# google/guetzli

Measured on AMD Instinct MI355X. Metric: MPix/s encoded at --quality 95, higher is better.
Workload: dtype f32+f64 (butteraugli), int32/int16 (DCT/quantize/entropy coding); 1 GPU; single 3840x2160 sRGB image, --quality 95 (BASELINE configs[2]), whole guetzli::Process per step (host RGB in, JPEG bytes out), 1 image per GPU per step; 12 timed steps after 5 warm-up between barrier + synchronise, max over ranks; images_per_gpu=1, steps=12, warmup=5, output_bytes=2895866

## Files before the change

guetzli_amd/csrc/api/chain.h:

```cpp
#pragma once

namespace {
static bool packed_blur(const gz_ctx* c) {
  if (c->cfg.blur_packed >= 0) return c->cfg.blur_packed != 0;
  return (size_t)c->w * c->h >= 1500000;
}
constexpr int kTileRows = 32;
constexpr int kSmallTileRows = 16;
static bool small_tiles(const gz_ctx* c) {
  if (c->cfg.tile_rows == 16) return true;
  if (c->cfg.tile_rows == 32) return false;
  return (size_t)c->w * c->h < 7000000;
}

template <int R, class Src, int NC>
int blur_h(gz_ctx* c, const SrcPack<Src, NC>& src, const PlanePack<NC>& dst,
           const BlurCfg& cfg) {
  if (cfg.r != R) { c->err = "blur radius mismatch"; return GZ_E_STATE; }
  const Taps<R> tp = taps_of<R>(cfg);
  const BorderScale bs = cfg.bx;
  const int w = c->w, h = c->h, pitch = c->pitch;
  if (packed_blur(c)) {
    dim3 grid(gz_div_up(c->w, HW), gz_div_up(c->h, HP), NC);
    GZ_LAUNCH((k_blur_h_pk<R, Src, NC>), grid, dim3(256), c->stream, src, dst, w, h, pitch, tp, bs, tp, bs);
  } else {
    dim3 grid(gz_div_up(c->w, HW), gz_div_up(c->h, HH), NC);
    GZ_LAUNCH((k_blur_h<R, Src, NC>), grid, dim3(256), c->stream, src, dst, w, h, pitch, tp, bs, tp, bs);
  }
  KCHK(c);
  return GZ_OK;
}

template <int R, int NC, class Post>
int blur_v(gz_ctx* c, const CPlanePack<NC>& src, const Post& post, const BlurCfg& cfg) {
  if (cfg.r != R) { c->err = "blur radius mismatch"; return GZ_E_STATE; }
  const Taps<R> tp = taps_of<R>(cfg);
  const BorderScale bs = cfg.by;
  const int w = c->w, h = c->h, pitch = c->pitch;
  const bool small = small_tiles(c);
  dim3 grid(gz_div_up(c->w, VW), gz_div_up(c->h, small ? kSmallTileRows : kTileRows));
  if (packed_blur(c)) {
    if (small) GZ_LAUNCH((k_blur_v_pk<R, NC, Post, kSmallTileRows>), grid, dim3(256), c->stream, src, post, w, h, pitch, tp, bs, tp, bs);
    else GZ_LAUNCH((k_blur_v_pk<R, NC, Post, kTileRows>), grid, dim3(256), c->stream, src, post, w, h, pitch, tp, bs, tp, bs);
  } else {
    if (small) GZ_LAUNCH((k_blur_v_compact<R, NC, Post, kSmallTileRows>), grid, dim3(256), c->stream, src, post, w, h, pitch, tp, bs, tp, bs);
    else GZ_LAUNCH((k_blur_v_compact<R, NC, Post, kTileRows>), grid, dim3(256), c->stream, src, post, w, h, pitch, tp, bs, tp, bs);
  }
  KCHK(c);
  return GZ_OK;
}

template <int R, class Src>
int blur_h_pair(gz_ctx* c, const SrcPack<Src, 2>& src, const PlanePack<2>& dst, const BlurCfg& cfg0,
                const BlurCfg& cfg1) {
  if (cfg0.r != R || cfg1.r != R) { c->err = "blur radius mismatch"; return GZ_E_STATE; }
  const Taps<R> t0 = taps_of<R>(cfg0), t1 = taps_of<R>(cfg1);
  const BorderScale b0 = cfg0.bx, b1 = cfg1.bx;
  const int w = c->w, h = c->h, pitch = c->pitch;
  if (packed_blur(c)) {
    dim3 grid(gz_div_up(c->w, HW), gz_div_up(c->h, HP), 2);
    GZ_LAUNCH((k_blur_h_pk<R, Src, 2, true>), grid, dim3(256), c->stream, src, dst, w, h, pitch, t0, b0, t1, b1);
  } else {
    dim3 grid(gz_div_up(c->w, HW), gz_div_up(c->h, HH), 2);
    GZ_LAUNCH((k_blur_h<R, Src, 2, true>), grid, dim3(256), c->stream, src, dst, w, h, pitch, t0, b0, t1, b1);
  }
  KCHK(c);
  return GZ_OK;
}
template <int R>
int blur_v_pair(gz_ctx* c, const CPlanePack<2>& src, const PostStore<2>& post, const BlurCfg& cfg0,
                const BlurCfg& cfg1) {
  if (cfg0.r != R || cfg1.r != R) { c->err = "blur radius mismatch"; return GZ_E_STATE; }
  const Taps<R> t0 = taps_of<R>(cfg0), t1 = taps_of<R>(cfg1);
  const BorderScale b0 = cfg0.by, b1 = cfg1.by;
  const int w = c->w, h = c->h, pitch = c->pitch;
  const bool small = small_tiles(c);
  dim3 grid(gz_div_up(c->w, VW), gz_div_up(c->h, small ? kSmallTileRows : kTileRows), 2);
  if (packed_blur(c)) {
    if (small) GZ_LAUNCH((k_blur_v_pk<R, 2, PostStore<2>, kSmallTileRows, true>), grid, dim3(256), c->stream, src, post, w, h, pitch, t0, b0, t1, b1);
    else GZ_LAUNCH((k_blur_v_pk<R, 2, PostStore<2>, kTileRows, true>), grid, dim3(256), c->stream, src, post, w, h, pitch, t0, b0, t1, b1);
  } else {
    if (small) GZ_LAUNCH((k_blur_v_compact<R, 2, PostStore<2>, kSmallTileRows, true>), grid, dim3(256), c->stream, src, post, w, h, pitch, t0, b0, t1, b1);
    else GZ_LAUNCH((k_blur_v_compact<R, 2, PostStore<2>, kTileRows, true>), grid, dim3(256), c->stream, src, post, w, h, pitch, t0, b0, t1, b1);
  }
  KCHK(c);
  return GZ_OK;
}

template <int R, int NC, class Src, class Post, bool BM = false>
int blur2d(gz_ctx* c, const SrcPack<Src, NC>& src, const Post& post, const BlurCfg& cfg,
           BlockMaxOut bm = BlockMaxOut{nullptr, nullptr, 0, nullptr}, int n_tiles = 0) {
  if (cfg.r != R) { c->err = "blur radius mismatch"; return GZ_E_STATE; }
  const Taps<R> tp = taps_of<R>(cfg);
  const BorderScale bx = cfg.bx, by = cfg.by;
  const int w = c->w, h = c->h, pitch = c->pitch;
  if (bm.tiles || (BM ? small_tiles(c) && (size_t)c->w * c->h < 1500000 : small_tiles(c))) {
    dim3 grid(gz_div_up(c->w, T2), gz_div_up(c->h, kSmallTileRows));
    if (bm.tiles) grid = dim3(n_tiles);
    GZ_LAUNCH((k_blur2d<R, NC, Src, Post, BM, kSmallTileRows>), grid, dim3(256), c->stream, src, post, w,
              h, pitch, tp, bx, by, bm);
  } else {
    dim3 grid(gz_div_up(c->w, T2), gz_div_up(c->h, kTileRows));
    if (bm.tiles) grid = dim3(n_tiles);
    GZ_LAUNCH((k_blur2d<R, NC, Src, Post, BM, kTileRows>), grid, dim3(256), c->stream, src, post, w,
              h, pitch, tp, bx, by, bm);
  }
  KCHK(c);
  return GZ_OK;
}

#define TRY(x) do { int rc_ = (x); if (rc_ != GZ_OK) return rc_; } while (0)

static int stage_reserve(gz_ctx* c, HostStage* st, size_t bytes, void** out) {
  if (!st->ev) HIPCHK(c, pool_event_create(&st->ev));
  if (st->busy) {
    HIPCHK(c, hipEventSynchronize(st->ev));
    st->busy = false;
  }
  if (bytes > st->cap) {
    if (st->h) (void)pool_host_free(st->h);
    st->h = nullptr;
    st->cap = 0;
    const size_t cap = bytes + bytes / 2 + 4096;
    HIPCHK(c, pool_host_malloc(&st->h, cap));
    st->cap = cap;
  }
  *out = st->h;
  return GZ_OK;
}
static int stage_sent(gz_ctx* c, HostStage* st, hipStream_t stream) {
  HIPCHK(c, hipEventRecord(st->ev, stream));
  st->busy = true;
  return GZ_OK;
}
static int result_buffer(gz_ctx* c, size_t bytes, void** out) {
  if (bytes > c->h_res_cap) {
    if (c->h_res) (void)pool_host_free(c->h_res);
    c->h_res = nullptr;
    c->h_res_cap = 0;
    const size_t cap = std::max<size_t>(bytes + bytes / 2, 1 << 16);
    HIPCHK(c, pool_host_malloc(&c->h_res, cap));
    c->h_res_cap = cap;
  }
  *out = c->h_res;
  return GZ_OK;
}
static void stage_free(HostStage* st) {
  if (st->ev) { (void)hipEventSynchronize(st->ev); pool_event_destroy(st->ev); }
  if (st->h) (void)pool_host_free(st->h);
  st->h = nullptr; st->ev = nullptr; st->cap = 0; st->busy = false;
}

int setup_blur_cfg(gz_ctx* c, BlurCfg* cfg, float sigma, float border_ratio) {
  make_taps_host(sigma, cfg);
  cfg->border_ratio = border_ratio;
  std::vector<float> xl, xh, yl, yh;
  border_scales_host(*cfg, c->w, &xl, &xh);
  border_scales_host(*cfg, c->h, &yl, &yh);
  const int r = cfg->r;
  if (cfg->d_scale == nullptr) HIPCHK(c, pool_malloc((void**)&cfg->d_scale, sizeof(float) * 4 * r));
  std::vector<float> all;
  all.insert(all.end(), xl.begin(), xl.end());
  all.insert(all.end(), xh.begin(), xh.end());
  all.insert(all.end(), yl.begin(), yl.end());
  all.insert(all.end(), yh.begin(), yh.end());
  HIPCHK(c, hipMemcpy(cfg->d_scale, all.data(), sizeof(float) * 4 * r, hipMemcpyHostToDevice));
  cfg->bx.lo = cfg->d_scale;
  cfg->bx.hi = cfg->d_scale + r;
  cfg->by.lo = cfg->d_scale + 2 * r;
  cfg->by.hi = cfg->d_scale + 3 * r;
  return GZ_OK;
}

int stage_opsin(gz_ctx* c, const int* tiles = nullptr, int n_tiles = 0) {
  SrcPack<SrcPlain, 3> s;
  for (int i = 0; i < 3; ++i) s.s[i].p = c->lin[i];
  PostOpsin post;
  for (int i = 0; i < 3; ++i) { post.lin[i] = c->lin[i]; post.xyb[i] = c->xyb[i]; }
  TRY((blur2d<2, 3, SrcPlain, PostOpsin>(c, s, post, c->blur[B_OPSIN], BlockMaxOut{nullptr, nullptr, 0, tiles}, n_tiles)));
  return GZ_OK;
}
static int opsin_tile_rows(const gz_ctx*) { return kSmallTileRows; }

int stage_separate(gz_ctx* c, Psycho* ps, bool side_b = false) {
  hipStream_t main_stream = c->stream;
  hipStream_t b_stream = side_b ? c->side_stream2 : c->stream;
  int rc = GZ_OK;
  if (side_b) {
    HIPCHK(c, hipEventRecord(c->ev_xyb, c->stream));
    HIPCHK(c, hipStreamWaitEvent(b_stream, c->ev_xyb, 0));
  }
  {
    c->stream = b_stream;
    SrcPack<SrcPlain, 1> s; PlanePack<1> t;
    s.s[0].p = c->xyb[2]; t.p[0] = c->distmap;
    rc = blur_h<16, SrcPlain, 1>(c, s, t, c->blur[B_LF]);
    c->stream = main_stream;
    TRY(rc);
  }
  {
    SrcPack<SrcPlain, 2> s; PlanePack<2> t; CPlanePack<2> ct;
    for (int i = 0; i < 2; ++i) { s.s[i].p = c->xyb[i]; t.p[i] = c->tmp[i]; ct.p[i] = c->tmp[i]; }
    TRY((blur_h<16, SrcPlain, 2>(c, s, t, c->blur[B_LF])));
    PostLFxy post;
    for (int i = 0; i < 2; ++i) { post.lf_raw[i] = c->lf_raw[i]; post.lf_vals[i] = ps->lfv[i]; }
    TRY((blur_v<16, 2, PostLFxy>(c, ct, post, c->blur[B_LF])));
  }
  if (side_b) {
    HIPCHK(c, hipEventRecord(c->ev_lfy, c->stream));
    HIPCHK(c, hipStreamWaitEvent(b_stream, c->ev_lfy, 0));
  }
  {
    c->stream = b_stream;
    CPlanePack<1> ct; ct.p[0] = c->distmap;
    PostLFb post; post.lf_raw_y = c->lf_raw[1]; post.lf_vals_b = ps->lfv[2];
    rc = blur_v<16, 1, PostLFb>(c, ct, post, c->blur[B_LF]);
    c->stream = main_stream;
    TRY(rc);
  }
  {
    SrcPack<SrcDiff, 2> s;
    for (int i = 0; i < 2; ++i) {
      s.s[i].a = c->xyb[i];
      s.s[i].b = c->lf_raw[i];
    }
    PostMF post;
    for (int i = 0; i < 2; ++i) {
      post.xyb[i] = c->xyb[i];
      post.lf_raw[i] = c->lf_raw[i];
      post.mf[i] = ps->mf[i];
      post.hf_pre[i] = c->hfp[i];
    }
    TRY((blur2d<8, 2, SrcDiff, PostMF>(c, s, post, c->blur[B_MF])));
  }
  {
    SrcPack<SrcPlain, 2> s;
    for (int i = 0; i < 2; ++i) s.s[i].p = c->hfp[i];
    PostHF post;
    for (int i = 0; i < 2; ++i) {
      post.hf_pre[i] = c->hfp[i];
      post.hf[i] = ps->hf[i];
      post.uhf[i] = ps->uhf[i];
    }
    post.lf_raw_y = c->lf_raw[1];
    TRY((blur2d<4, 2, SrcPlain, PostHF>(c, s, post, c->blur[B_HF])));
  }
  return GZ_OK;
}

int stage_mask_blurs(gz_ctx* c, const MaskPrePack& pk, hipStream_t other = nullptr) {
  dim3 grid(gz_div_up(c->w, 1024), c->h, 2);
  GZ_LAUNCH(k_mask_pre, grid, dim3(256), c->stream, pk, c->w, c->h, c->pitch);
  KCHK(c);
  if (other) {
    HIPCHK(c, hipEventRecord(c->ev_mask_pre, c->stream));
    HIPCHK(c, hipStreamWaitEvent(other, c->ev_mask_pre, 0));
  }
  {
    SrcPack<SrcPlain, 2> s; PlanePack<2> t; CPlanePack<2> ct;
    s.s[0].p = c->diffx; s.s[1].p = c->diffy;
    t.p[0] = c->tmp[1]; t.p[1] = c->tmp[2];
    ct.p[0] = c->tmp[1]; ct.p[1] = c->tmp[2];
    TRY((blur_h_pair<20, SrcPlain>(c, s, t, c->blur[B_MASKX], c->blur[B_MASKY1])));
    PostStore<2> post; post.out[0] = c->mxb; post.out[1] = c->myb2;
    TRY((blur_v_pair<20>(c, ct, post, c->blur[B_MASKX], c->blur[B_MASKY1])));
  }
  {
    SrcPack<SrcPlain, 1> s; s.s[0].p = c->diffy;
    PostStore<1> post; post.out[0] = c->myb1;
    hipStream_t here = c->stream;
    if (other) c->stream = other;
    const int rc = blur2d<5, 1, SrcPlain, PostStore<1>>(c, s, post, c->blur[B_MASKY0]);
    c->stream = here;
    TRY(rc);
  }
  return GZ_OK;
}

static void mask_in_psycho(const Psycho& p, MaskIn in[2]) {
  const double muls[4] = {0, 1.64178305129, 0.831081703362, 3.23680933546};
  for (int i = 0; i < 2; ++i) {
    in[i].a = muls[2 * i];
    in[i].b = muls[2 * i + 1];
    in[i].plain = 0;
    in[i].hf = p.hf[i];
    in[i].uhf = muls[2 * i] == 0 ? nullptr : p.uhf[i];
  }
}
int stage_mask_sup(gz_ctx* c, const MaskIn in[2], float* const out[2]) {
  MaskSupPack pk;
  for (int i = 0; i < 2; ++i) { pk.in[i] = in[i]; pk.out[i] = out[i]; }
  dim3 grid(gz_div_up(c->w, 1024), c->h, 2);
  GZ_LAUNCH(k_mask_sup, grid, dim3(256), c->stream, pk, c->w, c->h, c->pitch);
  KCHK(c);
  return GZ_OK;
}
MaskPrePack mask_pack_psycho(gz_ctx* c, const Psycho& b) {
  MaskPrePack pk;
  mask_in_psycho(b, pk.in1);
  pk.sup0[0] = c->sup0[0];
  pk.sup0[1] = c->sup0[1];
  pk.out[0] = c->diffx;
  pk.out[1] = c->diffy;
  return pk;
}
int ensure_pip(gz_ctx* c);
int mask_pack_plain(gz_ctx* c, const float* const a[2], const float* const b[2], MaskPrePack* pk) {
  MaskIn in0[2];
  for (int i = 0; i < 2; ++i) {
    in0[i] = {nullptr, a[i], 0.0, 1.0, 1};
    pk->in1[i] = {nullptr, b[i], 0.0, 1.0, 1};
  }
  TRY(ensure_pip(c));
  TRY(stage_mask_sup(c, in0, c->sup_scratch));
  pk->sup0[0] = c->sup_scratch[0];
  pk->sup0[1] = c->sup_scratch[1];
  pk->out[0] = c->diffx;
  pk->out[1] = c->diffy;
  return GZ_OK;
}

static bool single_stream_wanted(const gz_ctx* c) {
  if (c->cfg.single_stream >= 0) return c->cfg.single_stream != 0;
  return slots_taken(c->device) > 1;
}
static void choose_streams(gz_ctx* c) { c->single_now = single_stream_wanted(c); }
static bool single_stream(const gz_ctx* c) { return c->single_now; }
int fork_side_branch(gz_ctx* c, const Psycho& p0, const Psycho& p1) {
  if (single_stream(c)) {
    SrcPack<SrcSameNoise, 1> s; PlanePack<1> t; CPlanePack<1> ct;
    s.s[0].a = p0.hf[1]; s.s[0].b = p1.hf[1];
    t.p[0] = c->tmp[0]; ct.p[0] = c->tmp[0];
    TRY((blur_h<23, SrcSameNoise, 1>(c, s, t, c->blur[B_SN])));
    PostStore<1> post; post.out[0] = c->snb;
    TRY((blur_v<23, 1, PostStore<1>>(c, ct, post, c->blur[B_SN])));
    return stage_mask_blurs(c, mask_pack_psycho(c, p1));
  }
  HIPCHK(c, hipEventRecord(c->ev_fork, c->stream));
  HIPCHK(c, hipStreamWaitEvent(c->side_stream, c->ev_fork, 0));
  HIPCHK(c, hipStreamWaitEvent(c->side_stream2, c->ev_fork, 0));
  hipStream_t main_stream = c->stream;
  int rc = GZ_OK;
  c->stream = c->side_stream2;
  {
    SrcPack<SrcSameNoise, 1> s; PlanePack<1> t; CPlanePack<1> ct;
    s.s[0].a = p0.hf[1]; s.s[0].b = p1.hf[1];
    t.p[0] = c->tmp[0]; ct.p[0] = c->tmp[0];
    rc = blur_h<23, SrcSameNoise, 1>(c, s, t, c->blur[B_SN]);
    PostStore<1> post; post.out[0] = c->snb;
    if (rc == GZ_OK) rc = blur_v<23, 1, PostStore<1>>(c, ct, post, c->blur[B_SN]);
  }
  c->stream = c->side_stream;
  if (rc == GZ_OK) rc = stage_mask_blurs(c, mask_pack_psycho(c, p1), c->side_stream2);
  c->stream = main_stream;
  TRY(rc);
  HIPCHK(c, hipEventRecord(c->ev_join, c->side_stream));
  HIPCHK(c, hipEventRecord(c->ev_join2, c->side_stream2));
  return GZ_OK;
}
int join_mask_branch(gz_ctx* c) {
  if (single_stream(c)) return GZ_OK;
  HIPCHK(c, hipStreamWaitEvent(c->stream, c->ev_join, 0));
  HIPCHK(c, hipStreamWaitEvent(c->stream, c->ev_join2, 0));
  return GZ_OK;
}

int stage_diffmap(gz_ctx* c, const Psycho& p0, const Psycho& p1, bool want_block_max,
                  bool max_cleared = false, bool want_distmap = true, bool streams_chosen = false,
                  bool clear_in_combine = false) {
  if (!streams_chosen) choose_streams(c);
  const float hf_asymmetry_ = 0.8f;
  TRY(fork_side_branch(c, p0, p1));
  MaltaSpec ms[2][3];
  malta_specs(ms);
  dim3 mgrid(gz_div_up(c->w, MW), gz_div_up(c->h, MH), 2);
  MaltaArgs<3> ay, ax;
  for (int ch = 0; ch < 2; ++ch) {
    MaltaArgs<3>& a = ch ? ay : ax;
    a.pass[0] = {p0.uhf[ch], p1.uhf[ch], ms[ch][0].nm, ms[ch][0].lf};
    a.pass[1] = {p0.hf[ch], p1.hf[ch], ms[ch][1].nm, ms[ch][1].lf};
    a.pass[2] = {p0.mf[ch], p1.mf[ch], ms[ch][2].nm, ms[ch][2].lf};
    a.out = c->ac[ch];
  }
  GZ_LAUNCH((k_malta_rolled<3>), mgrid, dim3(256), c->stream, ay, ax, c->w, c->h, c->pitch);
  KCHK(c);
  TRY(join_mask_branch(c));
  {
    CombineArgs a;
    a.mask_x_blur = c->mxb; a.mask_y_blur1 = c->myb1; a.mask_y_blur2 = c->myb2;
    a.ac0 = c->ac[0]; a.ac1 = c->ac[1];
    a.lf0_x = p0.lfv[0]; a.lf1_x = p1.lfv[0];
    a.lf0_b = p0.lfv[2]; a.lf1_b = p1.lfv[2];
    a.luts = c->d_mask_luts;
    const double wmul1 = 32.4449876135;
    a.sn_blur = c->snb;
    a.hf0_y = p0.hf[1];
    a.hf1_y = p1.hf[1];
    a.w_sn = 884.809801415;
    a.w_0gt1 = (wmul1 * hf_asymmetry_) * 0.8;
    a.w_0lt1 = (wmul1 / hf_asymmetry_) * 0.8;
    a.out = c->dsq;
    for (int i = 0; i < 3; ++i) a.mask_out[i] = a.mask_dc_out[i] = nullptr;
    a.clear_word = clear_in_combine ? c->d_max_bits : nullptr;
    dim3 grid(gz_div_up(c->w, 1024), c->h);
    GZ_LAUNCH(k_combine, grid, dim3(256), c->stream, a, c->w, c->h, c->pitch);
    KCHK(c);
  }
  {
    SrcPack<SrcPlain, 1> s; s.s[0].p = c->dsq;
    PostDiffmapMix post; post.d = c->dsq; post.out = want_distmap ? c->distmap : nullptr;
    if (!max_cleared && !clear_in_combine) HIPCHK(c, hipMemsetAsync(c->d_max_bits, 0, sizeof(unsigned), c->stream));
    BlockMaxOut bm{want_block_max ? c->d_block_max : nullptr, c->d_max_bits, c->bw, nullptr};
    TRY((blur2d<3, 1, SrcPlain, PostDiffmapMix, true>(c, s, post, c->blur[B_FINAL], bm)));
  }
  return GZ_OK;
}

int enqueue_scan_offsets(gz_ctx* c, int which, hipStream_t stream, const unsigned* d_bits, int n,
                         unsigned long long* d_off) {
  const int max_tiles = gz_div_up(c->nb, kScanTile) + 1;
  const size_t bytes = (size_t)max_tiles * (8 + 8 + 4) + 64;
  if (!c->d_scan_state[which]) {
    HIPCHK(c, pool_malloc(&c->d_scan_state[which], bytes));
    HIPCHK(c, hipMemsetAsync(c->d_scan_state[which], 0, bytes, stream));
    c->scan_epoch[which] = 0;
  }
  char* base = (char*)c->d_scan_state[which];
  ScanState st;
  st.agg = (unsigned long long*)base;
  st.incl = st.agg + max_tiles;
  st.status = (unsigned*)(st.incl + max_tiles);
  st.ticket = st.status + max_tiles;
  unsigned ep = ++c->scan_epoch[which];
  if (ep >= 0x3fffffffu) {
    HIPCHK(c, hipMemsetAsync(c->d_scan_state[which], 0, bytes, stream));
    c->scan_epoch[which] = ep = 1;
  }
  if (n > max_tiles * kScanTile) { c->err = "scan larger than its scratch"; return GZ_E_STATE; }
  GZ_LAUNCH(k_scan_offsets, dim3(std::max(1, gz_div_up(n, kScanTile))), dim3(256), stream, d_bits, n, d_off, st, ep);
  KCHK(c);
  return GZ_OK;
}

int stage_chroma_samples(gz_ctx* c, const int16_t* d_coeffs) {
  if (!c->d_csamp) HIPCHK(c, pool_malloc((void**)&c->d_csamp, 2 * csamp_plane(c)));
  GZ_LAUNCH(k_chroma_samples, dim3(gz_div_up(c->nbc, kBlocksPerWG)), dim3(256), c->stream,
            d_coeffs + (size_t)c->coff[1] * 64, d_coeffs + (size_t)c->coff[2] * 64, c->cbw, c->nbc,
            c->d_csamp);
  KCHK(c);
  return GZ_OK;
}

int stage_reconstruct(gz_ctx* c, const int16_t* d_coeffs, float* lin0, uint8_t* srgb,
                      unsigned* clear_word = nullptr) {
  if (c->cfac == 2) {
    TRY(stage_chroma_samples(c, d_coeffs));
    GZ_LAUNCH(k_reconstruct420, dim3(c->bh * gz_div_up(c->bw, 8)), dim3(256), c->stream,
              d_coeffs, (const uint8_t*)c->d_csamp, c->w, c->h, c->bw, c->nb, c->cbw, c->cbh,
              c->pitch, c->plane, c->d_srgb_lut, lin0, srgb, clear_word);
    KCHK(c);
    return GZ_OK;
  }
  const int strips = gz_div_up(c->bw, kReconBlocks);
  int per = 4;
  while (per > 1 && (long)c->bh * gz_div_up(strips, per) < 2000) per >>= 1;
#ifdef GZ_EMU
  if (const char* e = getenv("GZ_EMU_RECON_STRIPS")) per = std::max(1, atoi(e));
#endif
  GZ_LAUNCH(k_reconstruct, dim3(c->bh * gz_div_up(strips, per)), dim3(256), c->stream,
            d_coeffs, c->w, c->h, c->bw, c->nb, c->pitch, c->plane, c->d_srgb_lut, lin0,
            srgb, clear_word, per);
  KCHK(c);
  return GZ_OK;
}

static std::atomic<unsigned long long> g_compares{0}, g_compares_patched{0}, g_patch_checks{0};
static std::atomic<unsigned long long> g_compares_ahead{0}, g_ahead_checks{0};
static int check_patched_planes(gz_ctx* c) {
  float* full = nullptr;
  unsigned* d_bad = nullptr;
  HIPCHK(c, pool_malloc((void**)&full, sizeof(float) * c->plane * 3));
  HIPCHK(c, pool_malloc((void**)&d_bad, sizeof(unsigned)));
  int rc = GZ_OK;
  unsigned bad = 0;
  do {
    if (hipMemsetAsync(d_bad, 0, sizeof(unsigned), c->stream) != hipSuccess) { rc = GZ_E_HIP; break; }
    const int strips = gz_div_up(c->bw, kReconBlocks);
    GZ_LAUNCH(k_reconstruct, dim3(c->bh * strips), dim3(256), c->stream, (const int16_t*)c->d_cand, c->w, c->h, c->bw, c->nb,
              c->pitch, c->plane, (const float*)c->d_srgb_lut, full, (uint8_t*)nullptr, (unsigned*)nullptr, 1);
    GZ_LAUNCH(k_count_differing_words, dim3(1024), dim3(256), c->stream, (const unsigned*)c->lin[0], (const unsigned*)full,
              (size_t)c->plane * 3, d_bad);
    if (hipMemcpyAsync(&bad, d_bad, sizeof(unsigned), hipMemcpyDeviceToHost, c->stream) != hipSuccess ||
        hipStreamSynchronize(c->stream) != hipSuccess) { rc = GZ_E_HIP; break; }
  } while (0);
  (void)pool_free(full);
  (void)pool_free(d_bad);
  TRY(rc);
  ++g_patch_checks;
  if (bad) { c->err = "patched linear planes differ from a full reconstruction"; return GZ_E_STATE; }
  return GZ_OK;
}

static int check_opsin_ahead(gz_ctx* c) {
  float* kept = nullptr;
  unsigned* d_bad = nullptr;
  HIPCHK(c, pool_malloc((void**)&kept, sizeof(float) * c->plane * 3));
  HIPCHK(c, pool_malloc((void**)&d_bad, sizeof(unsigned)));
  int rc = GZ_OK;
  unsigned bad = 0;
  do {
    if (hipMemsetAsync(d_bad, 0, sizeof(unsigned), c->stream) != hipSuccess) { rc = GZ_E_HIP; break; }
    for (int i = 0; i < 3 && rc == GZ_OK; ++i)
      if (hipMemcpyAsync(kept + (size_t)i * c->plane, c->xyb[i], sizeof(float) * c->plane, hipMemcpyDeviceToDevice, c->stream) != hipSuccess) rc = GZ_E_HIP;
    if (rc != GZ_OK) break;
    rc = stage_opsin(c);
    if (rc != GZ_OK) break;
    for (int i = 0; i < 3; ++i)
      GZ_LAUNCH(k_count_differing_words, dim3(1024), dim3(256), c->stream, (const unsigned*)c->xyb[i],
                (const unsigned*)(kept + (size_t)i * c->plane), (size_t)c->plane, d_bad);
    if (hipMemcpyAsync(&bad, d_bad, sizeof(unsigned), hipMemcpyDeviceToHost, c->stream) != hipSuccess ||
        hipStreamSynchronize(c->stream) != hipSuccess) { rc = GZ_E_HIP; break; }
  } while (0);
  (void)pool_free(kept);
  (void)pool_free(d_bad);
  TRY(rc);
  ++g_ahead_checks;
  if (bad) { c->err = "the opsin image kept ahead differs from the opsin blur of the whole planes"; return GZ_E_STATE; }
  return GZ_OK;
}

int enqueue_compare(gz_ctx* c, bool want_block_max, bool want_distmap = false, bool force_full = false) {
  want_distmap = want_distmap || c->cfg.store_distmap != 0;
  choose_streams(c);
  ++g_compares;
  const bool patched = !force_full && c->cfg.patch_reconstruct != 0 && c->lin_is_cand && c->cfac == 1;
  if (patched) {
    if (c->cfg.patch_reconstruct == 2) TRY(check_patched_planes(c));
    ++g_compares_patched;
  } else {
    TRY(stage_reconstruct(c, c->d_cand, c->lin[0], nullptr, c->d_max_bits));
    c->lin_is_cand = c->cfac == 1 && c->cfg.patch_reconstruct != 0 && (c->nb >= 8192 || c->cfg.patch_reconstruct == 2);
  }
  const bool ahead = patched && c->xyb_is_cand;
  c->xyb_is_cand = false;
  if (ahead) {
    if (c->cfg.patch_reconstruct == 2) TRY(check_opsin_ahead(c));
    ++g_compares_ahead;
  } else {
    TRY(stage_opsin(c));
  }
  TRY(stage_separate(c, &c->pi1, !single_stream(c)));
  TRY(stage_diffmap(c, c->pi0, c->pi1, want_block_max, !patched, want_distmap, true, patched));
  return GZ_OK;
}

int upload_planes(gz_ctx* c, const float* host, float* const* dev, int n) {
  for (int i = 0; i < n; ++i)
    HIPCHK(c, hipMemcpyAsync(dev[i], host + (size_t)i * c->w * c->h,
                             sizeof(float) * c->w * c->h, hipMemcpyHostToDevice, c->stream));
  return GZ_OK;
}
int download_plane(gz_ctx* c, const float* dev, float* host) {
  HIPCHK(c, hipMemcpyAsync(host, dev, sizeof(float) * c->w * c->h, hipMemcpyDeviceToHost,
                           c->stream));
  return GZ_OK;
}

int ensure_pip(gz_ctx* c) {
  if (c->have_pip) return GZ_OK;
  HIPCHK(c, pool_malloc((void**)&c->extra_arena, sizeof(float) * c->plane * 17));
  for (int i = 0; i < 17; ++i) c->free_planes.push_back(c->extra_arena + (size_t)i * c->plane);
  alloc_psycho(c, &c->pip);
  for (int i = 0; i < 3; ++i) { c->mask_out[i] = take_plane(c); c->mask_dc_out[i] = take_plane(c); }
  for (int i = 0; i < 2; ++i) c->sup_scratch[i] = take_plane(c);
  c->have_pip = true;
  return GZ_OK;
}


int ensure_block_mask(gz_ctx* c) {
  if (c->have_block_mask) return GZ_OK;
  TRY(ensure_pip(c));
  if (!c->d_block_mask) HIPCHK(c, pool_malloc((void**)&c->d_block_mask, sizeof(float) * 3 * c->nb));
  dim3 grid(gz_div_up(c->w, 256), c->h);
  c->lin_is_cand = c->xyb_is_cand = false;
  GZ_LAUNCH(k_linear_from_rgb8, grid, dim3(256), c->stream, c->d_rgb, c->w, c->h, c->pitch,
            c->plane, c->d_srgb_lut, c->lin[0]);
  KCHK(c);
  TRY(stage_opsin(c));
  MaskPrePack pk;
  {
    const float* const x2[2] = {c->xyb[0], c->xyb[1]};
    TRY(mask_pack_plain(c, x2, x2, &pk));
  }
  TRY(stage_mask_blurs(c, pk));
  CombineArgs ca;
  memset(&ca, 0, sizeof(ca));
  ca.mask_x_blur = c->mxb; ca.mask_y_blur1 = c->myb1; ca.mask_y_blur2 = c->myb2;
  ca.luts = c->d_mask_luts;
  for (int i = 0; i < 3; ++i) { ca.mask_out[i] = c->mask_out[i]; ca.mask_dc_out[i] = nullptr; }
  GZ_LAUNCH(k_combine, dim3(gz_div_up(c->w, 1024), c->h), dim3(256), c->stream, ca, c->w, c->h, c->pitch);
  KCHK(c);
  GZ_LAUNCH(k_gather_block_corners, dim3(gz_div_up(c->nb, 256)), dim3(256), c->stream,
            (const float*)c->mask_out[0], (const float*)c->mask_out[1],
            (const float*)c->mask_out[2], c->pitch, c->bw, c->nb, c->d_block_mask);
  KCHK(c);
  c->have_block_mask = true;
  return GZ_OK;
}

void rank_blocks(const int16_t* coeffs, const int16_t* orig, int nb, int new_model, int b0,
                 int b1, uint8_t* cnt, uint8_t* idx ) {
  static const uint8_t oldCsf[64] = {
      10, 10, 20, 40, 60, 70, 80, 90, 10, 20, 30, 60, 70, 80, 90, 90,
      20, 30, 60, 70, 80, 90, 90, 90, 40, 60, 70, 80, 90, 90, 90, 90,
      60, 70, 80, 90, 90, 90, 90, 90, 70, 80, 90, 90, 90, 90, 90, 90,
      80, 90, 90, 90, 90, 90, 90, 90, 90, 90, 90, 90, 90, 90, 90, 90};
  static const int zigzag[64] = {
      0, 1, 5, 6, 14, 15, 27, 28, 2, 4, 7, 13, 16, 26, 29, 42,
      3, 8, 12, 17, 25, 30, 41, 43, 9, 11, 18, 24, 31, 40, 44, 53,
      10, 19, 23, 32, 39, 45, 52, 54, 20, 22, 33, 38, 46, 51, 55, 60,
      21, 34, 37, 47, 50, 56, 59, 61, 35, 36, 48, 49, 57, 58, 62, 63};
  static const double kWeight[3] = {1.0, 0.22, 0.20};
  std::vector<std::pair<int, float> > order;
  order.reserve(192);
  for (int b = b0; b < b1; ++b) {
    order.clear();
    for (int ch = 0; ch < 3; ++ch) {
      const int16_t* blk = coeffs + ((size_t)ch * nb + b) * 64;
      const int16_t* ob = orig + ((size_t)ch * nb + b) * 64;
      for (int k = 1; k < 64; ++k) {
        if (blk[k] == 0) continue;
        const int i = ch * 64 + k;
        float score;
        if (new_model)
          score = abs((int)ob[k]) * kOrderCsf[i] + kOrderBias[i];
        else
          score = static_cast<float>((abs((int)ob[k]) - zigzag[k] / 64.0) * kWeight[ch] / oldCsf[k]);
        order.push_back(std::make_pair(i, score));
      }
    }
    std::sort(order.begin(), order.end(),
              [](const std::pair<int, float>& x, const std::pair<int, float>& y) {
                return x.second < y.second; });
    cnt[b] = (uint8_t)order.size();
    for (size_t i = 0; i < order.size(); ++i) idx[(size_t)b * 192 + i] = (uint8_t)order[i].first;
  }
}

void rank_all(const int16_t* coeffs, const int16_t* orig, int nb, int new_model,
              std::vector<int32_t>* off, std::vector<uint8_t>* idx) {
  std::vector<uint8_t> cnt(nb), wide((size_t)nb * 192);
  unsigned nt = std::thread::hardware_concurrency();
#if defined(__linux__)
  {
    cpu_set_t set;
    CPU_ZERO(&set);
    if (sched_getaffinity(0, sizeof(set), &set) == 0 && CPU_COUNT(&set) > 0) nt = (unsigned)CPU_COUNT(&set);
  }
#endif
  nt = std::max(1u, std::min(nt, 32u));
  if (nb < 4096) nt = 1;
  std::vector<std::thread> th;
  const int per = (nb + (int)nt - 1) / (int)nt;
  for (unsigned t = 0; t < nt; ++t) {
    const int b0 = (int)t * per, b1 = std::min(nb, b0 + per);
    if (b0 >= b1) break;
    th.emplace_back(rank_blocks, coeffs, orig, nb, new_model, b0, b1, cnt.data(), wide.data());
  }
  for (auto& t : th) t.join();
  off->resize(nb + 1);
  int total = 0;
  for (int b = 0; b < nb; ++b) { (*off)[b] = total; total += cnt[b]; }
  (*off)[nb] = total;
  idx->resize(total);
  for (int b = 0; b < nb; ++b)
    memcpy(idx->data() + (*off)[b], wide.data() + (size_t)b * 192, cnt[b]);
}

}
```

guetzli_amd/csrc/gz_kernels_diff.h:

```cpp
#pragma once
#include "gz_common.h"
#include "gz_kernels_block.h"
#include "gz_math.h"
#define GZ_TABLE GZ_CONST
#include "tables_generated.h"

namespace gz {

struct MaskIn {
  const float* uhf;
  const float* hf;
  double a, b;
  int plain;
  GZ_DEVFN float mix(float u, float v) const {
    if (plain) return v;
    if (uhf == nullptr) return (float)(b * (double)v);
    return (float)(a * (double)u + b * (double)v);
  }
  GZ_DEVFN float operator()(size_t idx) const {
    return mix(uhf ? GZ_LDG(uhf, idx) : 0.0f, GZ_LDG(hf, idx));
  }
  GZ_DEVFN gz_f4 load4(size_t idx) const {
    const gz_f4 v = GZ_LDG4(hf, idx);
    gz_f4 u = v, r;
    if (uhf) u = GZ_LDG4(uhf, idx);
#pragma unroll
    for (int i = 0; i < 4; ++i) r.v[i] = mix(u.v[i], v.v[i]);
    return r;
  }
};
struct MaskSupPack {
  MaskIn in[2];
  float* out[2];
};
struct MaskPrePack {
  const float* sup0[2];
  MaskIn in1[2];
  float* out[2];
};

struct MaskQuad { gz_f4 c, d; float r; };
GZ_DEVFN MaskQuad mask_quad(const MaskIn& a, int x, int y, int w, int h, int pitch) {
  const int y2 = y + 1 < h ? y + 1 : (y > 0 ? y - 1 : y);
  MaskQuad q;
  q.c = a.load4((size_t)y * pitch + x);
  q.d = a.load4((size_t)y2 * pitch + x);
  const int lane = (int)(threadIdx.x & 63);
  const float next = __uint_as_float((unsigned)__shfl((int)__float_as_uint(q.c.v[0]), lane + 1));
  if (lane != 63 && x + 7 < w) {
    q.r = next;
  } else {
    const int xr = x + 4 < w ? x + 4 : x + 2;
    q.r = a((size_t)y * pitch + xr);
  }
  return q;
}

__global__ __launch_bounds__(256) void k_mask_sup(MaskSupPack pk, int w, int h, int pitch) {
  const GzTile bid = gz_xcd_tile();
  const int x = (bid.x * (int)blockDim.x + (int)threadIdx.x) * 4, y = bid.y;
  if (x >= w || y >= h) return;
  const int c = bid.z;
  MaskIn a = pk.in[0];
  float* out = pk.out[0];
  if (c == 1) { a = pk.in[1]; out = pk.out[1]; }
  const int y2 = y + 1 < h ? y + 1 : (y > 0 ? y - 1 : y);
  if ((pitch & 3) == 0 && x + 3 < w) {
    const MaskQuad q = mask_quad(a, x, y, w, h, pitch);
    gz_f4 o;
#pragma unroll
    for (int k = 0; k < 4; ++k) o.v[k] = diff_sup(q.c.v[k], k < 3 ? q.c.v[k < 3 ? k + 1 : 3] : q.r, q.d.v[k]);
    GZ_STG4(out, (size_t)y * pitch + x, o);
    return;
  }
  for (int k = 0; k < 4 && x + k < w; ++k) {
    const int xx = x + k;
    const int x2 = xx + 1 < w ? xx + 1 : (xx > 0 ? xx - 1 : xx);
    const size_t i = (size_t)y * pitch + xx;
    out[i] = diff_sup(a(i), a((size_t)y * pitch + x2), a((size_t)y2 * pitch + xx));
  }
}

__global__ __launch_bounds__(256) void k_mask_pre(MaskPrePack pk, int w, int h, int pitch) {
  const GzTile bid = gz_xcd_tile();
  const int x = (bid.x * (int)blockDim.x + (int)threadIdx.x) * 4, y = bid.y;
  if (x >= w || y >= h) return;
  const int c = bid.z;
  MaskIn b = pk.in1[0];
  const float* sup0 = pk.sup0[0];
  float* out = pk.out[0];
  if (c == 1) { b = pk.in1[1]; sup0 = pk.sup0[1]; out = pk.out[1]; }
  const int y2 = y + 1 < h ? y + 1 : (y > 0 ? y - 1 : y);
  if ((pitch & 3) == 0 && x + 3 < w) {
    const size_t i = (size_t)y * pitch + x;
    const gz_f4 s0 = GZ_LDG4(sup0, i);
    const MaskQuad q = mask_quad(b, x, y, w, h, pitch);
    gz_f4 o;
#pragma unroll
    for (int k = 0; k < 4; ++k)
      o.v[k] = diff_from_sups(s0.v[k], diff_sup(q.c.v[k], k < 3 ? q.c.v[k < 3 ? k + 1 : 3] : q.r, q.d.v[k]));
    GZ_STG4(out, i, o);
    return;
  }
  for (int k = 0; k < 4 && x + k < w; ++k) {
    const int xx = x + k;
    const int x2 = xx + 1 < w ? xx + 1 : (xx > 0 ? xx - 1 : xx);
    const size_t i = (size_t)y * pitch + xx;
    out[i] = diff_from_sups(sup0[i], diff_sup(b(i), b((size_t)y * pitch + x2), b((size_t)y2 * pitch + xx)));
  }
}

constexpr int MW = 64;
constexpr int MH = 32;
constexpr int MPT = MH / 4;

struct MaltaPass {
  const float* p0;
  const float* p1;
  MaltaNorm nm;
  int lf;
};

template <bool LF>
GZ_DEVFN float malta_unit(const float (*t)[MW + 8], int ly, int lx) {
  float ret = 0.0f;
#pragma unroll
  for (int o = 0; o < 16; ++o) {
    float sum = 0.0f;
    if (LF) {
#pragma unroll
      for (int k = 0; k < 5; ++k) {
        const float v = t[ly + kMaltaLF[o][k][0]][lx + kMaltaLF[o][k][1]];
        sum = k == 0 ? v : sum + v;
      }
    } else {
#pragma unroll
      for (int k = 0; k < 9; ++k) {
        if (k < kMaltaHFCount[o]) {
          const float v = t[ly + kMaltaHF[o][k][0]][lx + kMaltaHF[o][k][1]];
          sum = k == 0 ? v : sum + v;
        }
      }
    }
    ret += sum * sum;
  }
  return ret;
}

template <int NPASS>
struct MaltaArgs {
  MaltaPass pass[NPASS];
  float* out;
};

template <int NPASS>
__global__ __launch_bounds__(256, 8) void k_malta_rolled(MaltaArgs<NPASS> a0, MaltaArgs<NPASS> a1, int w,
                                               int h, int pitch) {
  const GzTile bid = gz_xcd_tile();
  const MaltaArgs<NPASS>& a = bid.z ? a1 : a0;
  __shared__ __attribute__((aligned(16))) float tile[MH + 8][MW + 8];
  const int tx = threadIdx.x & 63, tg = threadIdx.x >> 6;
  const int x0 = bid.x * MW, y0 = bid.y * MH;
  __shared__ float accs[MPT][256];
#pragma unroll
  for (int i = 0; i < MPT; ++i) accs[i][threadIdx.x] = 0.0f;
  const bool vec = x0 >= 4 && x0 + MW + 4 <= w && (pitch & 3) == 0;
  for (int ps = 0; ps < NPASS; ++ps) {
    const MaltaPass P = a.pass[ps];
    MaltaNorm nm = P.nm;
    nm.norm1f = GZ_IN_VGPR(nm.norm1f);
    nm.norm2_0gt1 = GZ_IN_VGPR(nm.norm2_0gt1);
    nm.norm2_0lt1 = GZ_IN_VGPR(nm.norm2_0lt1);
    if (ps > 0) __syncthreads();
    if (vec) {
      constexpr int NV = (MH + 8) * ((MW + 8) / 4);
#pragma unroll 1
      for (int k = 0; k < (NV + 255) / 256; ++k) {
        const int i = 256 * k + (int)threadIdx.x;
        if (i < NV) {
          const int ry = i / ((MW + 8) / 4), q = i - ry * ((MW + 8) / 4);
          const int y = y0 - 4 + ry;
          gz_f4 v;
          v.v[0] = v.v[1] = v.v[2] = v.v[3] = 0.0f;
          if (y >= 0 && y < h) {
            const size_t idx = (size_t)y * pitch + (x0 - 4 + 4 * q);
            const gz_f4 u0 = GZ_LDG4(P.p0, idx), u1 = GZ_LDG4(P.p1, idx);
#pragma unroll
            for (int e = 0; e < 4; ++e) v.v[e] = malta_diff(u0.v[e], u1.v[e], nm);
          }
          *reinterpret_cast<gz_f4*>(&tile[ry][4 * q]) = v;
        }
      }
    } else {
      for (int i = threadIdx.x; i < (MH + 8) * (MW + 8); i += 256) {
        const int ry = i / (MW + 8), rx = i - ry * (MW + 8);
        const int x = x0 - 4 + rx, y = y0 - 4 + ry;
        float v = 0.0f;
        if (x >= 0 && x < w && y >= 0 && y < h) {
          const size_t idx = (size_t)y * pitch + x;
          v = malta_diff(GZ_LDG(P.p0, idx), GZ_LDG(P.p1, idx), nm);
        }
        tile[ry][rx] = v;
      }
    }
    __syncthreads();
#pragma unroll 1
    for (int i = 0; i < MPT; ++i) {
      const int ly = tg * MPT + i;
      const float r = P.lf ? malta_unit<true>(tile, ly + 4, tx + 4)
                           : malta_unit<false>(tile, ly + 4, tx + 4);
      accs[i][threadIdx.x] += r;
    }
  }
  const int x = x0 + tx;
  if (x >= w) return;
#pragma unroll
  for (int i = 0; i < MPT; ++i) {
    const int y = y0 + tg * MPT + i;
    if (y >= h) break;
    const size_t idx = (size_t)y * pitch + x;
    const float v = accs[i][threadIdx.x];
    GZ_STG(a.out, idx, v);
  }
}

struct CombineArgs {
  const float* mask_x_blur;
  const float* mask_y_blur1;
  const float* mask_y_blur2;
  const float* ac0;
  const float* ac1;
  const float* lf0_x;
  const float* lf1_x;
  const float* lf0_b;
  const float* lf1_b;
  const float* sn_blur;
  const float* hf0_y;
  const float* hf1_y;
  double w_sn, w_0gt1, w_0lt1;
  const double* luts;
  float* out;
  float* mask_out[3];
  float* mask_dc_out[3];
  unsigned* clear_word;
};

GZ_DEVFN void mask_p0p1(float bx, float by1, float by2, double* p0, double* p1) {
  const double muls0 = 0.207017089891, muls1 = 0.267138152891;
  const double normalizer = 1.0 / (muls0 + muls1);
  const float my = (float)(normalizer * (muls0 * (double)by1 + muls1 * (double)by2));
  const double s0 = (double)bx, s1 = (double)my;
  const double mul0 = 16.6963293877, mul1 = 2.1364621982;
  const double w00 = 36.4671237619, w11 = 2.1887170895, p1_to_p0 = 0.0513061271723;
  *p1 = (mul1 * w11) * s1;
  *p0 = (mul0 * w00) * s0 + p1_to_p0 * (*p1);
}

GZ_DEVFN float combine_px(const CombineArgs& a, size_t i, float mxb, float myb1, float myb2, float ac0,
                          float ac1_in, float lf0x, float lf1x, float lf0b, float lf1b, float snb,
                          float hf0y, float hf1y) {
  double p0, p1;
  mask_p0p1(mxb, myb1, myb2, &p0, &p1);
  const double w_ytob_hf = 0.086624184478, w_ytob_lf = 21.6804277046;
  const float m0 = (float)interp_lut512(a.luts, p0);
  const double my = interp_lut512(a.luts + 512, p1);
  const float m1 = (float)my;
  const float mdc0 = (float)interp_lut512(a.luts + 1024, p0);
  const double mdcy = interp_lut512(a.luts + 1536, p1);
  const float mdc1 = (float)mdcy;
  const float mdc2 = (float)(w_ytob_lf * mdcy);
  if (a.mask_out[0]) {
    a.mask_out[0][i] = m0;
    a.mask_out[1][i] = m1;
    a.mask_out[2][i] = (float)(w_ytob_hf * my);
  }
  if (a.mask_dc_out[0]) {
    a.mask_dc_out[0][i] = mdc0;
    a.mask_dc_out[1][i] = mdc1;
    a.mask_dc_out[2][i] = mdc2;
  }
  if (a.out == nullptr) return 0.0f;
  const float dc0 = l2diff_acc(0.0f, lf0x, lf1x, 1.01370836411);
  const float dc1 = 0.0f;
  const float dc2 = l2diff_acc(0.0f, lf0b, lf1b, 1.74566011615);
  const float ac2 = 0.0f;
  float ac1 = ac1_in;
  if (a.sn_blur) {
    const double d = (double)snb;
    ac1 = (float)((double)ac1 + (a.w_sn * d) * d);
    ac1 = l2diff_asym_acc(ac1, hf0y, hf1y, a.w_0gt1, a.w_0lt1);
  }
  const float m2 = (float)(w_ytob_hf * my);
  const float sdc = (dc0 * mdc0 + dc1 * mdc1) + dc2 * mdc2;
  const float sac = (ac0 * m0 + ac1 * m1) + ac2 * m2;
  const float v = sdc + sac;
  const float kInitialSlope = 100.0f;
  return v < (1.0f / (kInitialSlope * kInitialSlope)) ? kInitialSlope * v : sqrtf(v);
}

__global__ __launch_bounds__(256) void k_combine(CombineArgs a, int w, int h, int pitch) {
  const int x = (blockIdx.x * blockDim.x + threadIdx.x) * 4, y = blockIdx.y;
  if (a.clear_word && blockIdx.x == 0 && blockIdx.y == 0 && threadIdx.x == 0) *a.clear_word = 0u;
  if (x >= w || y >= h) return;
  const size_t i = (size_t)y * pitch + x;
  if ((pitch & 3) == 0 && x + 3 < w && a.out != nullptr) {
    const gz_f4 mxb = GZ_LDG4(a.mask_x_blur, i), myb1 = GZ_LDG4(a.mask_y_blur1, i), myb2 = GZ_LDG4(a.mask_y_blur2, i);
    const gz_f4 ac0 = GZ_LDG4(a.ac0, i), ac1 = GZ_LDG4(a.ac1, i);
    const gz_f4 lf0x = GZ_LDG4(a.lf0_x, i), lf1x = GZ_LDG4(a.lf1_x, i), lf0b = GZ_LDG4(a.lf0_b, i), lf1b = GZ_LDG4(a.lf1_b, i);
    gz_f4 snb = ac0, hf0y = ac0, hf1y = ac0;
    if (a.sn_blur) { snb = GZ_LDG4(a.sn_blur, i); hf0y = GZ_LDG4(a.hf0_y, i); hf1y = GZ_LDG4(a.hf1_y, i); }
    gz_f4 o;
#pragma unroll
    for (int k = 0; k < 4; ++k)
      o.v[k] = combine_px(a, i + k, mxb.v[k], myb1.v[k], myb2.v[k], ac0.v[k], ac1.v[k], lf0x.v[k], lf1x.v[k],
                          lf0b.v[k], lf1b.v[k], snb.v[k], hf0y.v[k], hf1y.v[k]);
    GZ_STG4(a.out, i, o);
    return;
  }
  for (int k = 0; k < 4 && x + k < w; ++k) {
    const size_t j = i + k;
    const bool full = a.out != nullptr;
    const float v = combine_px(a, j, a.mask_x_blur[j], a.mask_y_blur1[j], a.mask_y_blur2[j],
                               full ? a.ac0[j] : 0.0f, full ? a.ac1[j] : 0.0f,
                               full ? a.lf0_x[j] : 0.0f, full ? a.lf1_x[j] : 0.0f,
                               full ? a.lf0_b[j] : 0.0f, full ? a.lf1_b[j] : 0.0f,
                               full && a.sn_blur ? a.sn_blur[j] : 0.0f,
                               full && a.sn_blur ? a.hf0_y[j] : 0.0f, full && a.sn_blur ? a.hf1_y[j] : 0.0f);
    if (full) a.out[j] = v;
  }
}

__global__ void k_probe_arith(int op, const void* a, const void* b, const void* c, void* out,
                              int n) {
  const int i = blockIdx.x * blockDim.x + threadIdx.x;
  if (i >= n) return;
  switch (op) {
    case 0: ((float*)out)[i] = ((const float*)a)[i] / ((const float*)b)[i]; break;
    case 1: ((float*)out)[i] = sqrtf(((const float*)a)[i]); break;
    case 2: ((double*)out)[i] = ((const double*)a)[i] / ((const double*)b)[i]; break;
    case 3: ((double*)out)[i] = sqrt(((const double*)a)[i]); break;
    case 4: ((float*)out)[i] = ((const float*)a)[i] * ((const float*)b)[i] + ((const float*)c)[i]; break;
    case 5: ((double*)out)[i] = ((const double*)a)[i] * ((const double*)b)[i] + ((const double*)c)[i]; break;
    case 6: ((float*)out)[i] = (float)((const double*)a)[i]; break;
    default: break;
  }
}

}
```

Baseline: 35.15 MPix/s.

## Compute Malta filter four pixels per thread with row-swept vectorized LDS reads

Replaces the per-pixel Malta kernel with one where each thread computes a 1x4 strip of outputs. It sweeps the 9 stencil rows and loads 16-byte LDS vectors only for the segments each line group actually reads, with the tap tables made constexpr so that selection happens at compile time. The aim is to cut shared-memory load instructions and redundant reads across neighbouring pixels, and to use vectorized global stores. The cost is higher register pressure from the per-line partial sums, plus a swizzled thread-to-row mapping that adds complexity.

After: 35.38 MPix/s, median of 6. Within noise of the previous version (+0.7%).

```diff
diff --git a/guetzli_amd/csrc/api/chain.h b/guetzli_amd/csrc/api/chain.h
--- a/guetzli_amd/csrc/api/chain.h
+++ b/guetzli_amd/csrc/api/chain.h
@@ -382,7 +382,7 @@
     a.pass[2] = {p0.mf[ch], p1.mf[ch], ms[ch][2].nm, ms[ch][2].lf};
     a.out = c->ac[ch];
   }
-  GZ_LAUNCH((k_malta_rolled<3>), mgrid, dim3(256), c->stream, ay, ax, c->w, c->h, c->pitch);
+  GZ_LAUNCH((k_malta_rows<3>), mgrid, dim3(256), c->stream, ay, ax, c->w, c->h, c->pitch);
   KCHK(c);
   TRY(join_mask_branch(c));
   {
diff --git a/guetzli_amd/csrc/gz_kernels_diff.h b/guetzli_amd/csrc/gz_kernels_diff.h
--- a/guetzli_amd/csrc/gz_kernels_diff.h
+++ b/guetzli_amd/csrc/gz_kernels_diff.h
@@ -2,7 +2,8 @@
 #include "gz_common.h"
 #include "gz_kernels_block.h"
 #include "gz_math.h"
-#define GZ_TABLE GZ_CONST
+#include <utility>
+#define GZ_TABLE static constexpr
 #include "tables_generated.h"
 
 namespace gz {
@@ -112,7 +113,6 @@
 
 constexpr int MW = 64;
 constexpr int MH = 32;
-constexpr int MPT = MH / 4;
 
 struct MaltaPass {
   const float* p0;
@@ -121,30 +121,122 @@
   int lf;
 };
 
-template <bool LF>
-GZ_DEVFN float malta_unit(const float (*t)[MW + 8], int ly, int lx) {
-  float ret = 0.0f;
-#pragma unroll
-  for (int o = 0; o < 16; ++o) {
-    float sum = 0.0f;
-    if (LF) {
-#pragma unroll
-      for (int k = 0; k < 5; ++k) {
-        const float v = t[ly + kMaltaLF[o][k][0]][lx + kMaltaLF[o][k][1]];
-        sum = k == 0 ? v : sum + v;
-      }
-    } else {
-#pragma unroll
-      for (int k = 0; k < 9; ++k) {
-        if (k < kMaltaHFCount[o]) {
-          const float v = t[ly + kMaltaHF[o][k][0]][lx + kMaltaHF[o][k][1]];
-          sum = k == 0 ? v : sum + v;
+constexpr int malta_taps(bool lf, int o) { return lf ? kMaltaLFCount[o] : kMaltaHFCount[o]; }
+constexpr int malta_dy(bool lf, int o, int k) { return lf ? kMaltaLF[o][k][0] : kMaltaHF[o][k][0]; }
+constexpr int malta_dx(bool lf, int o, int k) { return lf ? kMaltaLF[o][k][1] : kMaltaHF[o][k][1]; }
+template <int... O>
+constexpr bool malta_reads(bool lf, int dy, int j) {
+  const int ls[] = {O...};
+  for (int o : ls)
+    for (int k = 0; k < malta_taps(lf, o); ++k)
+      if (malta_dy(lf, o, k) == dy && malta_dx(lf, o, k) + 7 >= 4 * j && malta_dx(lf, o, k) + 4 <= 4 * j + 3)
+        return true;
+  return false;
+}
+
+GZ_DEVFN gz_f4 malta_lds4(const float* p) {
+#ifdef GZ_EMU
+  return *reinterpret_cast<const gz_f4*>(p);
+#else
+  return gz_f4_from(*reinterpret_cast<const volatile __attribute__((address_space(3))) gz_vec4*>(
+      (const __attribute__((address_space(3))) float*)p));
+#endif
+}
+
+template <bool LF, int DY, int... O>
+GZ_DEVFN void malta_row(const float (*t)[MW + 8], int ly, int cx, float (&s)[sizeof...(O)][4]) {
+  constexpr int L[] = {O...};
+  constexpr bool rd[3] = {malta_reads<O...>(LF, DY, 0), malta_reads<O...>(LF, DY, 1),
+                          malta_reads<O...>(LF, DY, 2)};
+  float seg[12];
+#pragma unroll
+  for (int j = 0; j < 3; ++j) {
+    if (rd[j]) {
+      const gz_f4 v = malta_lds4(&t[ly + DY][cx + 4 * j]);
+#pragma unroll
+      for (int e = 0; e < 4; ++e) seg[4 * j + e] = v.v[e];
+    }
+  }
+#pragma unroll
+  for (int n = 0; n < (int)sizeof...(O); ++n) {
+#pragma unroll
+    for (int k = 0; k < 9; ++k) {
+      if (k < malta_taps(LF, L[n]) && malta_dy(LF, L[n], k) == DY) {
+#pragma unroll
+        for (int p = 0; p < 4; ++p) {
+          const float v = seg[4 + p + malta_dx(LF, L[n], k)];
+          s[n][p] = k == 0 ? v : s[n][p] + v;
         }
       }
     }
-    ret += sum * sum;
-  }
-  return ret;
+  }
+}
+
+template <bool LF, bool UP, int... O>
+struct MaltaSweep {
+  template <int... R>
+  static GZ_DEVFN void run(const float (*t)[MW + 8], int ly, int cx, float (&s)[sizeof...(O)][4],
+                           std::integer_sequence<int, R...>) {
+    (malta_row<LF, UP ? 4 - R : R - 4, O...>(t, ly, cx, s), ...);
+  }
+};
+template <bool LF, bool UP, int... O>
+GZ_DEVFN void malta_sweep(const float (*t)[MW + 8], int ly, int cx, float (&s)[sizeof...(O)][4]) {
+  MaltaSweep<LF, UP, O...>::run(t, ly, cx, s, std::make_integer_sequence<int, 9>());
+}
+
+template <int N>
+GZ_DEVFN void malta_add_squares(float (&ret)[4], const float (&s)[N][4], int n0 = 0, int n1 = N) {
+#pragma unroll
+  for (int n = n0; n < n1; ++n)
+#pragma unroll
+    for (int p = 0; p < 4; ++p) ret[p] += s[n][p] * s[n][p];
+}
+
+constexpr bool malta_monotone(bool lf, int o, bool up) {
+  for (int k = 1; k < malta_taps(lf, o); ++k)
+    if (up ? malta_dy(lf, o, k) > malta_dy(lf, o, k - 1) : malta_dy(lf, o, k) < malta_dy(lf, o, k - 1)) return false;
+  return true;
+}
+constexpr bool malta_sweeps_keep_order() {
+  for (int lf = 0; lf < 2; ++lf)
+    for (int o = 0; o < 16; ++o)
+      if (!malta_monotone(lf, o, o == 7 || o == 12)) return false;
+  return true;
+}
+static_assert(malta_sweeps_keep_order(), "a Malta line's taps do not run in the direction of its sweep");
+
+template <bool LF>
+GZ_DEVFN void malta_unit4(const float (*t)[MW + 8], int ly, int cx, float (&ret)[4]) {
+#pragma unroll
+  for (int p = 0; p < 4; ++p) ret[p] = 0.0f;
+  {
+    float s[4][4];
+    malta_sweep<LF, false, 0, 1, 2, 3>(t, ly, cx, s);
+    malta_add_squares(ret, s);
+  }
+  float s12[1][4];
+  {
+    float s[3][4];
+    malta_sweep<LF, false, 4, 5, 6>(t, ly, cx, s);
+    malta_add_squares(ret, s);
+    float su[2][4];
+    malta_sweep<LF, true, 7, 12>(t, ly, cx, su);
+    malta_add_squares(ret, su, 0, 1);
+#pragma unroll
+    for (int p = 0; p < 4; ++p) s12[0][p] = su[1][p];
+  }
+  {
+    float s[4][4];
+    malta_sweep<LF, false, 8, 9, 10, 11>(t, ly, cx, s);
+    malta_add_squares(ret, s);
+  }
+  malta_add_squares(ret, s12);
+  {
+    float s[3][4];
+    malta_sweep<LF, false, 13, 14, 15>(t, ly, cx, s);
+    malta_add_squares(ret, s);
+  }
 }
 
 template <int NPASS>
@@ -154,16 +246,19 @@
 };
 
 template <int NPASS>
-__global__ __launch_bounds__(256, 8) void k_malta_rolled(MaltaArgs<NPASS> a0, MaltaArgs<NPASS> a1, int w,
-                                               int h, int pitch) {
+__global__ __launch_bounds__(256, 8) void k_malta_rows(MaltaArgs<NPASS> a0, MaltaArgs<NPASS> a1, int w,
+                                                       int h, int pitch) {
   const GzTile bid = gz_xcd_tile();
   const MaltaArgs<NPASS>& a = bid.z ? a1 : a0;
   __shared__ __attribute__((aligned(16))) float tile[MH + 8][MW + 8];
-  const int tx = threadIdx.x & 63, tg = threadIdx.x >> 6;
+  __shared__ gz_f4 accs[2][256];
+  const int lane = threadIdx.x & 63;
+  const int q = ((lane >> 3) & 3) * 4 + (lane & 3);
+  const int r = (threadIdx.x >> 6) * 4 + (lane >> 5) * 2 + (((lane >> 4) ^ (lane >> 3) ^ (lane >> 2)) & 1);
   const int x0 = bid.x * MW, y0 = bid.y * MH;
-  __shared__ float accs[MPT][256];
-#pragma unroll
-  for (int i = 0; i < MPT; ++i) accs[i][threadIdx.x] = 0.0f;
+#pragma unroll
+  for (int i = 0; i < 2; ++i)
+    for (int p = 0; p < 4; ++p) accs[i][threadIdx.x].v[p] = 0.0f;
   const bool vec = x0 >= 4 && x0 + MW + 4 <= w && (pitch & 3) == 0;
   for (int ps = 0; ps < NPASS; ++ps) {
     const MaltaPass P = a.pass[ps];
@@ -178,17 +273,17 @@
       for (int k = 0; k < (NV + 255) / 256; ++k) {
         const int i = 256 * k + (int)threadIdx.x;
         if (i < NV) {
-          const int ry = i / ((MW + 8) / 4), q = i - ry * ((MW + 8) / 4);
+          const int ry = i / ((MW + 8) / 4), qq = i - ry * ((MW + 8) / 4);
           const int y = y0 - 4 + ry;
           gz_f4 v;
           v.v[0] = v.v[1] = v.v[2] = v.v[3] = 0.0f;
           if (y >= 0 && y < h) {
-            const size_t idx = (size_t)y * pitch + (x0 - 4 + 4 * q);
+            const size_t idx = (size_t)y * pitch + (x0 - 4 + 4 * qq);
             const gz_f4 u0 = GZ_LDG4(P.p0, idx), u1 = GZ_LDG4(P.p1, idx);
 #pragma unroll
             for (int e = 0; e < 4; ++e) v.v[e] = malta_diff(u0.v[e], u1.v[e], nm);
           }
-          *reinterpret_cast<gz_f4*>(&tile[ry][4 * q]) = v;
+          *reinterpret_cast<gz_f4*>(&tile[ry][4 * qq]) = v;
         }
       }
     } else {
@@ -205,22 +300,31 @@
     }
     __syncthreads();
 #pragma unroll 1
-    for (int i = 0; i < MPT; ++i) {
-      const int ly = tg * MPT + i;
-      const float r = P.lf ? malta_unit<true>(tile, ly + 4, tx + 4)
-                           : malta_unit<false>(tile, ly + 4, tx + 4);
-      accs[i][threadIdx.x] += r;
+    for (int i = 0; i < 2; ++i) {
+      float ret[4];
+      if (P.lf) malta_unit4<true>(tile, r + 16 * i + 4, 4 * q, ret);
+      else malta_unit4<false>(tile, r + 16 * i + 4, 4 * q, ret);
+      gz_f4 acc = accs[i][threadIdx.x];
+#pragma unroll
+      for (int p = 0; p < 4; ++p) acc.v[p] += ret[p];
+      accs[i][threadIdx.x] = acc;
     }
   }
-  const int x = x0 + tx;
+  const int x = x0 + 4 * q;
   if (x >= w) return;
 #pragma unroll
-  for (int i = 0; i < MPT; ++i) {
-    const int y = y0 + tg * MPT + i;
+  for (int i = 0; i < 2; ++i) {
+    const int y = y0 + r + 16 * i;
     if (y >= h) break;
     const size_t idx = (size_t)y * pitch + x;
-    const float v = accs[i][threadIdx.x];
-    GZ_STG(a.out, idx, v);
+    const gz_f4 v = accs[i][threadIdx.x];
+    if ((pitch & 3) == 0 && x + 3 < w) {
+      GZ_STG4(a.out, idx, v);
+    } else {
+#pragma unroll
+      for (int p = 0; p < 4; ++p)
+        if (x + p < w) GZ_STG(a.out, idx + p, v.v[p]);
+    }
   }
 }
 
```
